# radoslawkrolikowski/financial-market-data-analysis

Measured on AMD Instinct MI355X. Metric: train seq/sec + 3-class acc, biGRU on synthetic order-book, higher is better.
Workload: dtype bf16; 1 GPU; model=biGRU L2 H128 bidirectional, global_batch=8192, seq_len=120, n_features=96, parallelism=dp1, bench_config=repo

## Files before the change

fmda_amd/metrics.py:

```python
from typing import Tuple

import torch


def subset_accuracy(target: torch.Tensor, pred: torch.Tensor) -> torch.Tensor:
    t = target.to(torch.bool)
    p = pred.to(torch.bool)
    return (t == p).all(dim=1).float().mean()


def hamming(target: torch.Tensor, pred: torch.Tensor) -> torch.Tensor:
    t = target.to(torch.bool)
    p = pred.to(torch.bool)
    return (t != p).float().mean()


def fbeta_per_class(target: torch.Tensor, pred: torch.Tensor,
                    beta: float = 0.5) -> torch.Tensor:
    t = target.to(torch.float32)
    p = pred.to(torch.float32)
    tp = (t * p).sum(dim=0)
    fp = ((1 - t) * p).sum(dim=0)
    fn = (t * (1 - p)).sum(dim=0)
    b2 = beta * beta
    denom = (1 + b2) * tp + b2 * fn + fp
    fbeta = torch.where(denom > 0, (1 + b2) * tp / torch.clamp(denom, min=1e-38),
                        torch.zeros_like(denom))
    return fbeta
# ... 32 lines not shown
```

fmda_amd/ops/blas.py:

```python
import os


import torch

_TUNABLE_READY = False


def enable_tunableop() -> bool:
    global _TUNABLE_READY
    if _TUNABLE_READY or not torch.cuda.is_available():
        return _TUNABLE_READY
    try:
        tun = torch.cuda.tunable
        csv = os.path.join(os.path.dirname(__file__), "tunableop_gfx950.csv")
        tune = os.environ.get("FMDA_TUNE", "0") == "1"
        tun.set_filename(csv, insert_device_ordinal=False)
        tun.enable(True)
        tun.tuning_enable(tune)
        _TUNABLE_READY = True
    except Exception:
        _TUNABLE_READY = False
    return _TUNABLE_READY


def chunked_colsum(dg: torch.Tensor, chunks: int = 48) -> torch.Tensor:
    M, N = dg.shape
    c = chunks
    while c > 1 and M % c != 0:
        c //= 2
    if c <= 1:
        return dg.sum(dim=0, dtype=torch.float32)
    return dg.view(c, M // c, N).sum(dim=1, dtype=torch.float32).sum(dim=0)


def chunked_outer(dg: torch.Tensor, x: torch.Tensor,
                  chunks: int = 64, out_fp32: bool = False) -> torch.Tensor:
    parts = chunked_outer_parts(dg, x, chunks)
    if parts.shape[0] == 1:
        return parts[0].float() if out_fp32 else parts[0]
    s = parts.float().sum(dim=0)
    return s if out_fp32 else s.to(dg.dtype)


def chunked_outer_parts(dg: torch.Tensor, x: torch.Tensor,
                        chunks: int = 64) -> torch.Tensor:
    M, N = dg.shape
    K = x.shape[1]
    c = chunks
    while c > 1 and M % c != 0:
        c //= 2
    if c <= 1:
        return torch.matmul(dg.t(), x).unsqueeze(0)
    return torch.bmm(dg.view(c, M // c, N).transpose(1, 2),
                     x.view(c, M // c, K))
```

fmda_amd/ops/csrc/bindings.cpp:

```cpp
#include <torch/extension.h>
#include <ATen/hip/HIPContext.h>

#include <climits>
#include <cstdint>
#include <vector>

extern "C" int fmda_gru_fwd_launch(int is_bf16, int Hp, const void* gi,
                                   const void* w, const float* bhh, void* out,
                                   float* hlast, int B, int Tseq, int n_dir,
                                   const float* h0, void* out_drop,
                                   unsigned int drop_thr, float drop_scale,
                                   unsigned long long drop_seed,
                                   long gi_pitch, hipStream_t stream);
extern "C" int fmda_gru_fwd_cs_launch(const void* gi, const void* w,
                                      const float* bhh, void* out,
                                      float* hlast, void* hpub,
                                      unsigned int* cnt, int B, int Tseq,
                                      int n_dir, void* out_drop,
                                      unsigned int drop_thr,
                                      float drop_scale,
                                      unsigned long long drop_seed,
                                      long gi_pitch, hipStream_t stream);
extern "C" int fmda_gru_bwd_cs_launch(const void* gi, const void* w,
                                      const void* wt, const float* bhh,
// ... 63 lines not shown
                                    float* logits, float* sig,
                                    float* loss_sum, int B, int K, int C,
                                    hipStream_t stream);
extern "C" int fmda_head_bwd_launch(int is_bf16, const float* sig,
                                    const float* y, const float* wgt,
                                    const float* pw, const float* gscale,
                                    const void* W, float* dlogits, void* dx,
                                    int B, int K, int C, hipStream_t stream);
extern "C" int fmda_gru_bwd_db_rows(int is_bf16, int Hp, int B,
                                    int column_split);
extern "C" int fmda_gru_db_reduce_launch(const float* part, int rows,
                                         int n_dir, int Hp, float* dbhh,
                                         float* dbih, hipStream_t stream);
extern "C" int fmda_opt_norm2_launch(const void* chunks, int n_chunks,
                                     float* out, hipStream_t stream);
extern "C" int fmda_pack_gru_layer_launch(
        int is_bf16, const float* const* masters, void* w_ih_cat,
        void* b_ih_cat, void* w_hh_cat, float* b_hh_cat, void* wt, int D,
        int H, int Hp, int F, hipStream_t stream);
extern "C" int fmda_finalize_gru_wgrads_launch(
        int part_bf16, const void* part_ih, int c_ih, const void* part_hh,
        int c_hh, float* const* grads, int D, int H, int Hp, int F,
        hipStream_t stream);
extern "C" int fmda_head_fwd_master_launch(
        int is_bf16, const void* x, const float* W, const float* bias,
        const float* y, const float* wgt, const float* pw, float* logits,
        float* sig, float* loss_sum, int B, int K, int C,
        hipStream_t stream);
extern "C" int fmda_head_bwd_master_launch(
        int is_bf16, const float* sig, const float* y, const float* wgt,
        const float* pw, const float* gscale, const float* W,
        float* dlogits, void* dx, int B, int K, int C, hipStream_t stream);
extern "C" int fmda_normalize_table_launch(
        int out_bf16, const float* x, const float* xmin, const float* xmax,
        void* y, long N, int F, hipStream_t stream);
extern "C" int fmda_window_batch_launch(
        int is_bf16, const void* table, const long* starts, void* out,
        long B, long Tlen, long F, int mode, unsigned int thr, float scale,
        unsigned long long seed, hipStream_t stream);
extern "C" int fmda_head_wgrads_slabs(int B);
extern "C" int fmda_head_wgrads_launch(
        int is_bf16, const float* dlogits, const void* x, float* dw_part,
        float* db_part, float* dW, float* db, int B, int K, int C,
        hipStream_t stream);
namespace fmda_ckpt {
void save_state_dict(const std::string& path,
                     const std::vector<std::string>& keys,
                     const std::vector<torch::Tensor>& tensors);
std::vector<std::pair<std::string, torch::Tensor>> load_state_dict(
        const std::string& path);
}

extern "C" int fmda_opt_adam_launch(const void* chunks, int n_chunks,
                                    const float* norm2, float clip, float lr,
                                    float beta1, float beta2, float eps,
// ... 617 lines not shown
                        torch::IntArrayRef({3 * H, H}) &&
                    masters[4 * d + 2].sizes() == torch::IntArrayRef({3 * H}) &&
                    masters[4 * d + 3].sizes() == torch::IntArrayRef({3 * H}),
                    "pack_gru_layer: master shapes disagree");
        for (int k = 0; k < 4; ++k)
            ptrs[4 * d + k] = masters[4 * d + k].data_ptr<float>();
    }
    const bool bf16 = compute_dtype_is_bf16(dtype);
    auto opt = masters[0].options().dtype(dtype);
    auto w_ih_cat = torch::empty({D * 3 * Hp, F}, opt);
    auto b_ih_cat = torch::empty({D * 3 * Hp}, opt);
    auto w_hh_cat = torch::empty({D, 3 * Hp, Hp}, opt);
    auto b_hh_cat = torch::empty({D, 3 * Hp}, masters[0].options());
    auto wt = torch::empty({D, Hp, 3 * Hp}, opt);
    auto stream = at::hip::getCurrentHIPStream();
    int rc = fmda_pack_gru_layer_launch(
        bf16 ? 1 : 0, ptrs, w_ih_cat.data_ptr(), b_ih_cat.data_ptr(),
        w_hh_cat.data_ptr(), b_hh_cat.data_ptr<float>(), wt.data_ptr(),
        (int)D, (int)H, (int)Hp, (int)F, stream.stream());
    TORCH_CHECK(rc == 0, "pack_gru_layer launch failed");
    return {w_ih_cat, b_ih_cat, w_hh_cat, b_hh_cat, wt};
}

std::vector<torch::Tensor> finalize_gru_wgrads(torch::Tensor part_ih,
                                               torch::Tensor part_hh,
                                               int64_t D, int64_t H,
                                               int64_t Hp) {
    TORCH_CHECK(part_ih.is_cuda() && part_hh.is_cuda() &&
                part_ih.is_contiguous() && part_hh.is_contiguous() &&
                part_ih.dim() == 3 && part_hh.dim() == 3,
                "finalize_gru_wgrads: partials must be contiguous (c, N, K) "
                "GPU tensors");
    TORCH_CHECK(part_ih.scalar_type() == part_hh.scalar_type(),
                "finalize_gru_wgrads: partial dtypes disagree");
    const bool bf16 = compute_dtype_is_bf16(part_ih.scalar_type());
    TORCH_CHECK((D == 1 || D == 2) && H >= 1 && H <= Hp,
                "finalize_gru_wgrads: bad D / H / Hp");
    const int64_t F = part_ih.size(2);
    TORCH_CHECK(part_ih.size(1) == D * 3 * Hp &&
                part_hh.size(1) == D * 3 * Hp && part_hh.size(2) == D * Hp,
                "finalize_gru_wgrads: partial shapes disagree with D / Hp");
    auto f32 = part_ih.options().dtype(torch::kFloat32);
    std::vector<torch::Tensor> grads;
    float* ptrs[4] = {};
    for (int64_t d = 0; d < D; ++d) {
        grads.push_back(torch::empty({3 * H, F}, f32));
        grads.push_back(torch::empty({3 * H, H}, f32));
        ptrs[2 * d] = grads[2 * d].data_ptr<float>();
        ptrs[2 * d + 1] = grads[2 * d + 1].data_ptr<float>();
    }
    auto stream = at::hip::getCurrentHIPStream();
    int rc = fmda_finalize_gru_wgrads_launch(
        bf16 ? 1 : 0, part_ih.data_ptr(), (int)part_ih.size(0),
        part_hh.data_ptr(), (int)part_hh.size(0), ptrs, (int)D, (int)H,
        (int)Hp, (int)F, stream.stream());
    TORCH_CHECK(rc == 0, "finalize_gru_wgrads launch failed");
    return grads;
}

std::vector<torch::Tensor> head_loss_fwd_master(
        torch::Tensor x, torch::Tensor W, torch::Tensor b, torch::Tensor y,
        torch::Tensor wgt, torch::Tensor pw) {
    TORCH_CHECK(x.is_cuda() && x.is_contiguous() && x.dim() == 2);
    const bool bf16 = compute_dtype_is_bf16(x.scalar_type());
    check_f32_cuda(W, "head W"); check_f32_cuda(b, "head b");
    check_f32_cuda(y, "head y"); check_f32_cuda(wgt, "head weight");
    check_f32_cuda(pw, "head pos_weight");
    const int B = x.size(0), K = x.size(1), C = W.size(0);
    TORCH_CHECK(W.size(1) == K && b.numel() == C && y.numel() == (int64_t)B * C
                && wgt.numel() == C && pw.numel() == C,
                "head_loss_fwd_master: shape mismatch");
    auto f32 = x.options().dtype(torch::kFloat32);
    auto logits = torch::empty({B, C}, f32);
    auto sig = torch::empty({B, C}, f32);
    auto part = torch::empty({((int64_t)B * C + 255) / 256}, f32);
    auto stream = at::hip::getCurrentHIPStream();
    int rc = fmda_head_fwd_master_launch(
        bf16 ? 1 : 0, x.data_ptr(), W.data_ptr<float>(), b.data_ptr<float>(),
        y.data_ptr<float>(), wgt.data_ptr<float>(), pw.data_ptr<float>(),
        logits.data_ptr<float>(), sig.data_ptr<float>(),
        part.data_ptr<float>(), B, K, C, stream.stream());
    TORCH_CHECK(rc == 0, "head fwd (master) launch failed");
    return {logits, sig, part.sum().reshape({1})};
}

std::vector<torch::Tensor> head_loss_bwd_master(
        torch::Tensor sig, torch::Tensor y, torch::Tensor wgt,
        torch::Tensor pw, torch::Tensor gscale, torch::Tensor W,
        torch::ScalarType xdtype) {
    check_f32_cuda(sig, "head sig"); check_f32_cuda(y, "head y");
    check_f32_cuda(wgt, "head weight"); check_f32_cuda(pw, "head pos_weight");
    check_f32_cuda(gscale, "head gscale"); check_f32_cuda(W, "head W");
    const int B = sig.size(0), C = sig.size(1), K = W.size(1);
    TORCH_CHECK(W.size(0) == C && y.numel() == sig.numel() &&
                wgt.numel() == C && pw.numel() == C && gscale.numel() == 1,
                "head_loss_bwd_master: shape mismatch");
    const bool bf16 = compute_dtype_is_bf16(xdtype);
    auto dlogits = torch::empty_like(sig);
    auto dx = torch::empty({B, K}, sig.options().dtype(xdtype));
    auto stream = at::hip::getCurrentHIPStream();
    int rc = fmda_head_bwd_master_launch(
        bf16 ? 1 : 0, sig.data_ptr<float>(), y.data_ptr<float>(),
        wgt.data_ptr<float>(), pw.data_ptr<float>(),
        gscale.data_ptr<float>(), W.data_ptr<float>(),
        dlogits.data_ptr<float>(), dx.data_ptr(), B, K, C, stream.stream());
    TORCH_CHECK(rc == 0, "head bwd (master) launch failed");
    return {dlogits, dx};
}

std::vector<torch::Tensor> head_wgrads(torch::Tensor dlogits,
                                       torch::Tensor x) {
    check_f32_cuda(dlogits, "head dlogits");
    TORCH_CHECK(x.is_cuda() && x.is_contiguous() && x.dim() == 2 &&
                dlogits.dim() == 2 && dlogits.size(0) == x.size(0),
                "head_wgrads: shape mismatch");
    const bool bf16 = compute_dtype_is_bf16(x.scalar_type());
    const int B = x.size(0), K = x.size(1), C = dlogits.size(1);
    const int64_t n_slabs = fmda_head_wgrads_slabs(B);
    auto f32 = dlogits.options();
    auto dw_part = torch::empty({n_slabs, C, K}, f32);
    auto db_part = torch::empty({n_slabs, C}, f32);
    auto dW = torch::empty({C, K}, f32);
    auto db = torch::empty({C}, f32);
    auto stream = at::hip::getCurrentHIPStream();
    int rc = fmda_head_wgrads_launch(
        bf16 ? 1 : 0, dlogits.data_ptr<float>(), x.data_ptr(),
        dw_part.data_ptr<float>(), db_part.data_ptr<float>(),
        dW.data_ptr<float>(), db.data_ptr<float>(), B, K, C,
        stream.stream());
    TORCH_CHECK(rc == 0, "head_wgrads launch failed");
// ... 29 lines not shown
    m.def("spatial_dropout_fused", &spatial_dropout_fused,
          "channel (Dropout2d) dropout over (B, T, F) without permutes");
    m.def("ingest_row", &ingest_row,
          "streaming ingest: shift GPU window ring + normalize new row");
    m.def("pool_concat_infer", &pool_concat_infer,
          "fused [dirsum(h_last) | max | avg] concat for inference");
    m.def("head_sigmoid", &head_sigmoid,
          "linear head + sigmoid emitting probabilities");
    m.def("pool_fwd", &pool_fwd, "fused dirsum+max/avg pooling forward",
          py::arg("out"), py::arg("n_dir"), py::arg("act_dtype") = false,
          py::arg("serial") = false);
    m.def("pool_features_fwd", &pool_features_fwd,
          "[dirsum(h_last) | max | avg] features + argmax in one kernel",
          py::arg("out"), py::arg("h_last"));
    m.def("pool_features_bwd", &pool_features_bwd,
          "d_out and d_hlast of pool_features_fwd in one kernel",
          py::arg("dfeat"), py::arg("amax"), py::arg("T"), py::arg("n_dir"));
    m.def("pool_bwd", &pool_bwd, "fused pooling backward (d_out assembly)");
    m.def("head_loss_fwd", &head_loss_fwd, "fused head GEMM + BCE loss");
    m.def("head_loss_bwd", &head_loss_bwd, "fused head/loss backward");
    m.def("pack_gru_layer", &pack_gru_layer,
          "fp32 masters -> padded compute-dtype layer weights (+ W_hh^T)");
    m.def("finalize_gru_wgrads", &finalize_gru_wgrads,
          "split-K partials -> master-shaped fp32 dW_ih / dW_hh");
    m.def("head_loss_fwd_master", &head_loss_fwd_master,
          "fused head GEMM + BCE loss reading the fp32 master W / b");
    m.def("head_loss_bwd_master", &head_loss_bwd_master,
          "fused head/loss backward reading the fp32 master W");
    m.def("head_wgrads", &head_wgrads,
          "head dW / db in fp32, two-stage fixed-order batch reduction");
    m.def("fused_clip_adam", &fused_clip_adam,
          "fused multi-tensor grad-clip + Adam step");
    m.def("save_state_dict_native", &fmda_ckpt::save_state_dict,
          "write a torch.load-compatible zip state_dict (native C++)");
    m.def("load_state_dict_native", &fmda_ckpt::load_state_dict,
          "read a torch.save zip state_dict (native C++)");
}
```

fmda_amd/ops/csrc/glue_kernels.hip:

```cpp
#include <hip/hip_runtime.h>
#include <hip/hip_bf16.h>

#include <cstdint>

#include "dropout_common.h"

#define FMDA_DEV __device__ __forceinline__

namespace fmda {
namespace {

#define FMDA_LOG2E 1.4426950408889634f

FMDA_DEV float fast_exp2(float x) { return __builtin_amdgcn_exp2f(x); }
FMDA_DEV float fast_rcp(float x) { return __builtin_amdgcn_rcpf(x); }
FMDA_DEV float sigmoidf(float x) {
    return fast_rcp(1.0f + fast_exp2(-x * FMDA_LOG2E));
}

template <typename T> FMDA_DEV float to_f32(T v);
template <> FMDA_DEV float to_f32<float>(float v) { return v; }
template <> FMDA_DEV float to_f32<__hip_bfloat16>(__hip_bfloat16 v) {
    return __bfloat162float(v);
}
template <typename T> FMDA_DEV T from_f32(float v);
template <> FMDA_DEV float from_f32<float>(float v) { return v; }
template <> FMDA_DEV __hip_bfloat16 from_f32<__hip_bfloat16>(float v) {
    return __float2bfloat16(v);
}
template <typename T> FMDA_DEV float round_to(float v) {
    return to_f32<T>(from_f32<T>(v));
}

struct GruMasters {
    const float* w_ih[2];
    const float* w_hh[2];
    const float* b_ih[2];
    const float* b_hh[2];
};

template <typename T>
__global__ void pack_gru_layer_kernel(GruMasters m, T* __restrict__ w_ih_cat,
                                      T* __restrict__ b_ih_cat,
                                      T* __restrict__ w_hh_cat,
                                      float* __restrict__ b_hh_cat,
                                      T* __restrict__ wt, int D, int H,
                                      int Hp, int F) {
    const long G3 = 3L * Hp;
    const long n_ih = (long)D * G3 * F;
    const long n_hh = (long)D * G3 * Hp;
    const long n_b = (long)D * G3;
    const long total = n_ih + 2 * n_hh + 2 * n_b;
    const long stride = (long)gridDim.x * blockDim.x;
    for (long i = (long)blockIdx.x * blockDim.x + threadIdx.x; i < total;
         i += stride) {
// ... 58 lines not shown
    const long r = idx % per_dir;
    float acc = 0.0f;
    if (r < n_ih) {
        const int row = (int)(r / F), col = (int)(r % F);
        const long prow = (long)d * 3 * Hp + (long)(row / H) * Hp + row % H;
        const PT* p = part_ih + prow * F + col;
        const long cs = (long)D * 3 * Hp * F;
#pragma unroll 8
        for (int k = 0; k < c_ih; ++k) acc += to_f32<PT>(p[k * cs]);
        o.dw_ih[d][r] = acc;
    } else {
        const long q = r - n_ih;
        const int row = (int)(q / H), col = (int)(q % H);
        const long prow = (long)d * 3 * Hp + (long)(row / H) * Hp + row % H;
        const long pitch = (long)D * Hp;
        const PT* p = part_hh + prow * pitch + (long)d * Hp + col;
        const long cs = (long)D * 3 * Hp * pitch;
#pragma unroll 8
        for (int k = 0; k < c_hh; ++k) acc += to_f32<PT>(p[k * cs]);
        o.dw_hh[d][q] = acc;
    }
}

template <typename T>
__global__ void head_fwd_master_kernel(const T* __restrict__ x,
                                       const float* __restrict__ W,
                                       const float* __restrict__ bias,
                                       const float* __restrict__ y,
                                       const float* __restrict__ wgt,
                                       const float* __restrict__ pw,
                                       float* __restrict__ logits,
                                       float* __restrict__ sig,
                                       float* __restrict__ loss_sum, int B,
                                       int K, int C) {
    const int idx = blockIdx.x * blockDim.x + threadIdx.x;
    float l = 0.0f;
    if (idx < B * C) {
        const int r = idx / C, c = idx % C;
        const T* xr = x + (long)r * K;
        const float* wr = W + (long)c * K;
        float acc = round_to<T>(bias[c]);
        for (int k = 0; k < K; ++k)
            acc += to_f32<T>(xr[k]) * round_to<T>(wr[k]);
        logits[idx] = acc;
        const float s = sigmoidf(acc);
        sig[idx] = s;
        const float yy = y[idx];
        const float m = acc > 0.0f ? acc : 0.0f;
        const float lse = m + __builtin_logf(fast_exp2(-m * FMDA_LOG2E) +
                                             fast_exp2((acc - m) * FMDA_LOG2E));
        const float log_s = acc - lse;
        const float log_1ms = -lse;
        l = -wgt[c] * (pw[c] * yy * log_s + (1.0f - yy) * log_1ms);
    }
    __shared__ float red[4];
    float v = l;
    v += __shfl_xor(v, 1); v += __shfl_xor(v, 2); v += __shfl_xor(v, 4);
    v += __shfl_xor(v, 8); v += __shfl_xor(v, 16); v += __shfl_xor(v, 32);
    if ((threadIdx.x & 63) == 0) red[threadIdx.x >> 6] = v;
    __syncthreads();
    if (threadIdx.x == 0) {
        float t = 0.0f;
        for (int w = 0; w < (int)(blockDim.x >> 6); ++w) t += red[w];
        loss_sum[blockIdx.x] = t;
    }
}

template <typename T>
__global__ void head_bwd_master_kernel(const float* __restrict__ sig,
                                       const float* __restrict__ y,
                                       const float* __restrict__ wgt,
                                       const float* __restrict__ pw,
                                       const float* __restrict__ gscale,
                                       const float* __restrict__ W,
                                       float* __restrict__ dlogits,
                                       T* __restrict__ dx, int B, int K,
                                       int C) {
    const int idx = blockIdx.x * blockDim.x + threadIdx.x;
    if (idx >= B * K) return;
    const int r = idx / K, k = idx % K;
    const float g = *gscale / (float)(B * C);
    float acc = 0.0f;
    for (int c = 0; c < C; ++c) {
        const float s = sig[r * C + c];
        const float yy = y[r * C + c];
        const float dl = g * wgt[c] * (s * (1.0f - yy + pw[c] * yy) -
                                       pw[c] * yy);
        if (k == 0) dlogits[r * C + c] = dl;
        acc += dl * round_to<T>(W[(long)c * K + k]);
    }
    dx[idx] = from_f32<T>(acc);
}

constexpr int HEAD_SLAB = 64;

struct CompSum {
    float s = 0.0f, c = 0.0f;
    FMDA_DEV void add(float v) {
#pragma clang fp contract(off)
        const float t = s + v;
        c += fabsf(s) >= fabsf(v) ? (s - t) + v : (v - t) + s;
        s = t;
    }
    FMDA_DEV float value() const { return s + c; }
};

template <typename T>
__global__ void head_wgrads_stage1_kernel(const float* __restrict__ dlogits,
                                          const T* __restrict__ x,
                                          float* __restrict__ dw_part,
                                          float* __restrict__ db_part, int B,
// ... 19 lines not shown
    if (k == 0) db_part[slab * C + c] = db.value();
}

__global__ void head_wgrads_stage2_kernel(const float* __restrict__ dw_part,
                                          const float* __restrict__ db_part,
                                          float* __restrict__ dW,
                                          float* __restrict__ db, int n_slabs,
                                          int K, int C) {
    const int idx = blockIdx.x * blockDim.x + threadIdx.x;
    const int n_w = C * K;
    if (idx >= n_w + C) return;
    CompSum a;
    if (idx < n_w) {
#pragma unroll 8
        for (int s = 0; s < n_slabs; ++s) a.add(dw_part[(long)s * n_w + idx]);
        dW[idx] = a.value();
    } else {
        const int c = idx - n_w;
        for (int s = 0; s < n_slabs; ++s) a.add(db_part[s * C + c]);
        db[c] = a.value();
    }
}

template <typename T>
__global__ void normalize_table_kernel(const float* __restrict__ x,
                                       const float* __restrict__ xmin,
                                       const float* __restrict__ xmax,
                                       T* __restrict__ y, long total, int F) {
    const long stride = (long)gridDim.x * blockDim.x;
    for (long i = (long)blockIdx.x * blockDim.x + threadIdx.x; i < total;
         i += stride) {
        const int f = (int)(i % F);
        float v = x[i];
        if (v != v) v = 0.0f;
        else if (v == __builtin_inff()) v = 3.402823466e+38f;
        else if (v == -__builtin_inff()) v = -3.402823466e+38f;
        const float mn = xmin[f];
        y[i] = from_f32<T>(__fdiv_rn(__fsub_rn(v, mn), __fsub_rn(xmax[f], mn)));
    }
}

struct alignas(16) chunk16 { unsigned int u[4]; };

template <int LB>
FMDA_DEV void load16(void* dst, const void* src) {
    if constexpr (LB == 16) {
        *(chunk16*)dst = *(const chunk16*)src;
    } else if constexpr (LB == 8) {
        ((uint2*)dst)[0] = ((const uint2*)src)[0];
        ((uint2*)dst)[1] = ((const uint2*)src)[1];
    } else {
        static_assert(LB == 4, "load16: LB is 16, 8 or 4");
#pragma unroll
        for (int k = 0; k < 4; ++k)
            ((unsigned int*)dst)[k] = ((const unsigned int*)src)[k];
    }
}

template <typename T, int LB, int MODE>
__global__ void window_batch_kernel(const T* __restrict__ table,
                                    const long* __restrict__ starts,
                                    T* __restrict__ out, long n, long TF,
                                    int F, unsigned int thr, float scale,
                                    unsigned long long seed) {
    constexpr int V = 16 / (int)sizeof(T);
// ... 116 lines not shown

extern "C" int fmda_finalize_gru_wgrads_launch(
        int part_bf16, const void* part_ih, int c_ih, const void* part_hh,
        int c_hh, float* const* grads, int D, int H, int Hp, int F,
        hipStream_t stream) {
    GruWgrads o = {};
    for (int d = 0; d < D; ++d) {
        o.dw_ih[d] = grads[2 * d + 0];
        o.dw_hh[d] = grads[2 * d + 1];
    }
    const long total = (long)D * 3 * H * ((long)F + H);
    const dim3 grid((unsigned)((total + 255) / 256));
    if (part_bf16)
        finalize_gru_wgrads_kernel<__hip_bfloat16><<<grid, 256, 0, stream>>>(
            (const __hip_bfloat16*)part_ih, c_ih,
            (const __hip_bfloat16*)part_hh, c_hh, o, D, H, Hp, F);
    else
        finalize_gru_wgrads_kernel<float><<<grid, 256, 0, stream>>>(
            (const float*)part_ih, c_ih, (const float*)part_hh, c_hh, o, D,
            H, Hp, F);
    return launch_ok();
}

extern "C" int fmda_head_fwd_master_launch(
        int is_bf16, const void* x, const float* W, const float* bias,
        const float* y, const float* wgt, const float* pw, float* logits,
        float* sig, float* loss_sum, int B, int K, int C,
        hipStream_t stream) {
    const dim3 grid((B * C + 255) / 256);
    if (is_bf16)
        head_fwd_master_kernel<__hip_bfloat16><<<grid, 256, 0, stream>>>(
            (const __hip_bfloat16*)x, W, bias, y, wgt, pw, logits, sig,
            loss_sum, B, K, C);
    else
        head_fwd_master_kernel<float><<<grid, 256, 0, stream>>>(
            (const float*)x, W, bias, y, wgt, pw, logits, sig, loss_sum, B,
            K, C);
    return launch_ok();
}

extern "C" int fmda_head_bwd_master_launch(
        int is_bf16, const float* sig, const float* y, const float* wgt,
        const float* pw, const float* gscale, const float* W,
        float* dlogits, void* dx, int B, int K, int C, hipStream_t stream) {
    const dim3 grid((B * K + 255) / 256);
    if (is_bf16)
        head_bwd_master_kernel<__hip_bfloat16><<<grid, 256, 0, stream>>>(
            sig, y, wgt, pw, gscale, W, dlogits, (__hip_bfloat16*)dx, B, K,
            C);
    else
        head_bwd_master_kernel<float><<<grid, 256, 0, stream>>>(
            sig, y, wgt, pw, gscale, W, dlogits, (float*)dx, B, K, C);
    return launch_ok();
}

extern "C" int fmda_normalize_table_launch(
        int out_bf16, const float* x, const float* xmin, const float* xmax,
        void* y, long N, int F, hipStream_t stream) {
    const long total = N * (long)F;
    if (total == 0) return 0;
    const long blocks = (total + 255) / 256;
    const dim3 grid((unsigned)(blocks < 4096 ? blocks : 4096));
    if (out_bf16)
        normalize_table_kernel<__hip_bfloat16><<<grid, 256, 0, stream>>>(
            x, xmin, xmax, (__hip_bfloat16*)y, total, F);
    else
        normalize_table_kernel<float><<<grid, 256, 0, stream>>>(
            x, xmin, xmax, (float*)y, total, F);
    return launch_ok();
}

extern "C" int fmda_window_batch_load_bytes(const void* table, long TF,
                                            long F, int es) {
    if (TF % (16 / es) != 0) return 0;
    const uintptr_t addr = (uintptr_t)table;
// ... 59 lines not shown
```

fmda_amd/ops/interface.py:

```python
import os
from typing import List, Optional, Tuple

import torch

from . import load_extension
from .blas import (chunked_colsum, chunked_outer, chunked_outer_parts,
                   enable_tunableop)

_ALLOWED_HP = [32, 64, 128, 256, 512]


def _pad_h(H: int) -> int:
    for hp in _ALLOWED_HP:
        if H <= hp:
            return hp
    raise ValueError(f"hidden size {H} > {_ALLOWED_HP[-1]} not supported")


def _glue_mode() -> int:
    return {"0": 0, "2": 2}.get(os.environ.get("FMDA_NATIVE_GLUE", "1"), 1)


def _native_glue() -> bool:
    return _glue_mode() >= 1


def _native_reductions() -> bool:
    return _glue_mode() == 2


def _fp32_cuda(*tensors) -> bool:
    return all(t.is_cuda and t.dtype == torch.float32 for t in tensors)


def _pad_gate_rows(w: torch.Tensor, H: int, Hp: int) -> torch.Tensor:
    if H == Hp:
        return w
    shape = list(w.shape)
    shape[0] = 3 * Hp
    out = w.new_zeros(shape)
    for g in range(3):
        out[g * Hp:g * Hp + H] = w[g * H:(g + 1) * H]
    return out


def _pad_cols(w: torch.Tensor, H: int, Hp: int) -> torch.Tensor:
    if H == Hp:
        return w
    shape = list(w.shape)
    shape[-1] = Hp
    out = w.new_zeros(shape)
# ... 262 lines not shown

    @staticmethod
    def backward(ctx, dloss, _dlogits):
        ext = load_extension()
        x2d, W, y, wgt, pw, sig = ctx.saved_tensors
        dlogits, dx = ext.head_loss_bwd(sig, y, wgt, pw,
                                        dloss.reshape(1).float().contiguous(),
                                        W, x2d.dtype)
        dl = dlogits.to(x2d.dtype)
        dW = chunked_outer(dl, x2d)
        db = dlogits.sum(dim=0).to(W.dtype)
        return dx, dW, db, None, None, None


class _HeadLossMaster(torch.autograd.Function):

    @staticmethod
    def forward(ctx, x2d, W, b, y, wgt, pw):
        ext = load_extension()
        ctx.native_reductions = _native_reductions()
        x2d = x2d.contiguous()
        W = W.contiguous()
        y, wgt, pw = y.contiguous(), wgt.contiguous(), pw.contiguous()
        logits, sig, loss_sum = ext.head_loss_fwd_master(
            x2d, W, b.contiguous(), y, wgt, pw)
        B, C = logits.shape
        loss = (loss_sum / float(B * C)).reshape(())
        ctx.save_for_backward(x2d, W, y, wgt, pw, sig)
        ctx.mark_non_differentiable(logits)
        return loss, logits

    @staticmethod
    def backward(ctx, dloss, _dlogits):
        ext = load_extension()
        x2d, W, y, wgt, pw, sig = ctx.saved_tensors
        dlogits, dx = ext.head_loss_bwd_master(
            sig, y, wgt, pw, dloss.reshape(1).float().contiguous(), W,
            x2d.dtype)
        if ctx.native_reductions:
            dW, db = ext.head_wgrads(dlogits, x2d)
        else:
            dW = chunked_outer(dlogits.to(x2d.dtype), x2d).to(W.dtype)
            db = dlogits.sum(dim=0).to(x2d.dtype).to(W.dtype)
        return dx, dW, db, None, None, None


def fused_head_loss(x2d, weight, bias, y, wgt, pw):
    if (_native_glue() and x2d.is_cuda and _fp32_cuda(weight, bias)
            and x2d.dtype in (torch.bfloat16, torch.float32)):
        return _HeadLossMaster.apply(x2d, weight, bias, y.float(),
                                     wgt.float(), pw.float())
    Wc = weight.to(x2d.dtype)
    bc = bias.to(x2d.dtype)
    return _HeadLoss.apply(x2d, Wc, bc, y.float(), wgt.float(), pw.float())


def _unpad_gate_rows(w, H, Hp):
    if H == Hp:
        return w
    return torch.cat([w[g * Hp:g * Hp + H] for g in range(3)], dim=0)


class _BiGRULayer(torch.autograd.Function):

# ... 2 lines not shown
                w_ih1, w_hh1, b_ih1, b_hh1, out_drop_p=0.0,
                out_drop_seed=0, h0=None):
        ext = load_extension()
        D = 2 if w_ih1 is not None else 1
        H = w_hh0.shape[1]
        dtype = x.dtype
        B, T, F = x.shape
        params = [(w_ih0, w_hh0, b_ih0, b_hh0)]
        if D == 2:
            params.append((w_ih1, w_hh1, b_ih1, b_hh1))
        with torch.no_grad():
            w_ih_cat, b_ih_cat, w_hh_cat, b_hh_cat, wt = _pack_layer(
                params, H, Hp, dtype)
        x2d = x.reshape(B * T, F)
        gi = torch.addmm(b_ih_cat, x2d, w_ih_cat.t()).view(B, T, -1)
        h0c = h0.detach().contiguous() if h0 is not None else None
        res = ext.gru_fwd(gi, w_hh_cat, b_hh_cat, h0c, out_drop_p,
                          out_drop_seed)
        out, h_last = res[0], res[1]
        ctx.save_for_backward(x2d, w_ih_cat, w_hh_cat, b_hh_cat, gi, out, wt)
        ctx.h0 = h0c
        ctx.meta = (D, H, Hp, out_drop_p, out_drop_seed)
        ctx.native_reductions = _native_reductions()
        ctx.set_materialize_grads(False)
        if len(res) > 2:
            return out, h_last, res[2]
        return out, h_last

    @staticmethod
    def backward(ctx, d_out, d_hlast, d_outdrop=None):
        ext = load_extension()
        x2d, w_ih_cat, w_hh_cat, b_hh_cat, gi, out, wt = ctx.saved_tensors
        D, H, Hp, drop_p, drop_seed = ctx.meta
        need_dx = ctx.needs_input_grad[0]
        if drop_p > 0:
            assert d_out is None, "unexpected grad on raw out with fused dropout"
            d_out = d_outdrop
        if d_out is None:
            d_out = torch.zeros_like(out)
        if d_hlast is None:
            d_hlast = out.new_zeros(
                (w_hh_cat.shape[0], out.shape[0], Hp), dtype=torch.float32)
        d_out = d_out.contiguous().to(gi.dtype)
        d_hlast = d_hlast.contiguous().float()
        h0c = ctx.h0
        res = ext.gru_bwd(gi, w_hh_cat, b_hh_cat, out, d_out, d_hlast,
                          drop_p, drop_seed, h0c, wt)
        dgi, dgh, dh0_out, dbhh, dbih = res[:5]
        dgh0 = res[5] if len(res) > 5 else None
        M = dgi.shape[0] * dgi.shape[1]
        dx = None
        if need_dx:
            dx = torch.matmul(dgi.reshape(M, -1), w_ih_cat)
            dx = dx.view(dgi.shape[0], dgi.shape[1], -1)
        dh0_grad = dh0_out if h0c is not None else None

        if wt is not None and ctx.native_reductions and dgh0 is None:
            wg = ext.finalize_gru_wgrads(
                chunked_outer_parts(dgi.reshape(M, -1), x2d),
                chunked_outer_parts(dgh.reshape(M, -1), out.reshape(M, -1)),
                D, H, Hp)
            wgrads = [(wg[2 * d], wg[2 * d + 1]) for d in range(D)]
        else:
            cross = chunked_outer(dgh.reshape(M, -1), out.reshape(M, -1),
                                  out_fp32=True)
            if dgh0 is not None:
                for d in range(D):
                    cross[d * 3 * Hp:(d + 1) * 3 * Hp,
                          d * Hp:(d + 1) * Hp] += dgh0[d].float().t() @ h0c[d]
            dwih_cat = chunked_outer(dgi.reshape(M, -1), x2d, out_fp32=True)
            wgrads = []
            for d in range(D):
                dwih = dwih_cat[d * 3 * Hp:(d + 1) * 3 * Hp]
                dwhh = cross[d * 3 * Hp:(d + 1) * 3 * Hp,
                             d * Hp:(d + 1) * Hp].contiguous()
                wgrads.append((_unpad_gate_rows(dwih, H, Hp),
                               _unpad_gate_rows(dwhh, H, Hp)[:, :H]))

        grads = [wgrads[d] + (_unpad_gate_rows(dbih[d], H, Hp),
                              _unpad_gate_rows(dbhh[d], H, Hp))
                 for d in range(D)]
        if D == 1:
            grads.append((None, None, None, None))
        (a0, b0, c0, e0), (a1, b1, c1, e1) = grads
# ... 166 lines not shown
```

Baseline: 1.064 million seq/s.

## Add fused eager-order wgrad reductions, staged head forward, and native subset accuracy

Adds custom kernels that reduce the 64 split-K GEMM partials into master-shaped fp32 GRU and head weight gradients in one pass. The summation order mirrors the eager chunked sum so results stay bit-identical, and it replaces the chain of float cast, sum, slice and unpad ops. The head forward gains an LDS-staged variant that tiles x and W into shared memory, and the head backward can emit a bf16 copy of dlogits directly. Subset accuracy becomes a single-block kernel. These trim launch count and memory traffic in the glue path, at the cost of several shape-specific code paths.

```diff
diff --git a/fmda_amd/metrics.py b/fmda_amd/metrics.py
--- a/fmda_amd/metrics.py
+++ b/fmda_amd/metrics.py
@@ -4,6 +4,17 @@
 
 
 def subset_accuracy(target: torch.Tensor, pred: torch.Tensor) -> torch.Tensor:
+    if (target.is_cuda and pred.is_cuda and pred.dtype == torch.bool
+            and target.dtype in (torch.float32, torch.bool)
+            and target.dim() == 2 and target.shape == pred.shape
+            and target.device == pred.device
+            and 1 <= target.shape[0] <= 65536
+            and 1 <= target.shape[1] <= 65536
+            and target.is_contiguous() and pred.is_contiguous()):
+        from .ops import load_extension
+        from .ops.interface import _native_glue
+        if _native_glue():
+            return load_extension().subset_accuracy(target, pred)
     t = target.to(torch.bool)
     p = pred.to(torch.bool)
     return (t == p).all(dim=1).float().mean()
diff --git a/fmda_amd/ops/blas.py b/fmda_amd/ops/blas.py
--- a/fmda_amd/ops/blas.py
+++ b/fmda_amd/ops/blas.py
@@ -42,13 +42,18 @@
     return s if out_fp32 else s.to(dg.dtype)
 
 
+def split_chunks(M: int, chunks: int = 64) -> int:
+    c = chunks
+    while c > 1 and M % c != 0:
+        c //= 2
+    return max(c, 1)
+
+
 def chunked_outer_parts(dg: torch.Tensor, x: torch.Tensor,
                         chunks: int = 64) -> torch.Tensor:
     M, N = dg.shape
     K = x.shape[1]
-    c = chunks
-    while c > 1 and M % c != 0:
-        c //= 2
+    c = split_chunks(M, chunks)
     if c <= 1:
         return torch.matmul(dg.t(), x).unsqueeze(0)
     return torch.bmm(dg.view(c, M // c, N).transpose(1, 2),
diff --git a/fmda_amd/ops/csrc/bindings.cpp b/fmda_amd/ops/csrc/bindings.cpp
--- a/fmda_amd/ops/csrc/bindings.cpp
+++ b/fmda_amd/ops/csrc/bindings.cpp
@@ -109,15 +109,27 @@
         int part_bf16, const void* part_ih, int c_ih, const void* part_hh,
         int c_hh, float* const* grads, int D, int H, int Hp, int F,
         hipStream_t stream);
+extern "C" int fmda_finalize_gru_wgrads_eager_launch(
+        int part_bf16, const void* part_ih, const void* part_hh,
+        float* const* grads, int D, int H, int Hp, int F,
+        hipStream_t stream);
+extern "C" int fmda_eager_sum_chunks();
+extern "C" int fmda_head_wgrads_eager_launch(
+        int is_bf16, const void* parts, const float* db_sum, float* dW,
+        float* db, int K, int C, hipStream_t stream);
+extern "C" int fmda_subset_accuracy_launch(
+        int target_is_float, const void* target, const void* pred,
+        float* out, int B, int C, hipStream_t stream);
 extern "C" int fmda_head_fwd_master_launch(
         int is_bf16, const void* x, const float* W, const float* bias,
         const float* y, const float* wgt, const float* pw, float* logits,
-        float* sig, float* loss_sum, int B, int K, int C,
+        float* sig, float* loss_sum, int B, int K, int C, int staged,
         hipStream_t stream);
 extern "C" int fmda_head_bwd_master_launch(
         int is_bf16, const float* sig, const float* y, const float* wgt,
         const float* pw, const float* gscale, const float* W,
-        float* dlogits, void* dx, int B, int K, int C, hipStream_t stream);
+        float* dlogits, void* dlogits_t, void* dx, int B, int K, int C,
+        hipStream_t stream);
 extern "C" int fmda_normalize_table_launch(
         int out_bf16, const float* x, const float* xmin, const float* xmax,
         void* y, long N, int F, hipStream_t stream);
@@ -781,10 +793,19 @@
     return {w_ih_cat, b_ih_cat, w_hh_cat, b_hh_cat, wt};
 }
 
+bool eager_sum_applies(torch::Tensor parts) {
+    if (parts.dim() != 3 || parts.size(0) != fmda_eager_sum_chunks())
+        return false;
+    const int64_t outputs = parts.size(1) * parts.size(2);
+    return outputs >= 512 && outputs % 4 == 0;
+}
+
+
 std::vector<torch::Tensor> finalize_gru_wgrads(torch::Tensor part_ih,
                                                torch::Tensor part_hh,
                                                int64_t D, int64_t H,
-                                               int64_t Hp) {
+                                               int64_t Hp,
+                                               bool eager_order) {
     TORCH_CHECK(part_ih.is_cuda() && part_hh.is_cuda() &&
                 part_ih.is_contiguous() && part_hh.is_contiguous() &&
                 part_ih.dim() == 3 && part_hh.dim() == 3,
@@ -809,17 +830,27 @@
         ptrs[2 * d + 1] = grads[2 * d + 1].data_ptr<float>();
     }
     auto stream = at::hip::getCurrentHIPStream();
-    int rc = fmda_finalize_gru_wgrads_launch(
-        bf16 ? 1 : 0, part_ih.data_ptr(), (int)part_ih.size(0),
-        part_hh.data_ptr(), (int)part_hh.size(0), ptrs, (int)D, (int)H,
-        (int)Hp, (int)F, stream.stream());
+    int rc;
+    if (eager_order) {
+        TORCH_CHECK(eager_sum_applies(part_ih) && eager_sum_applies(part_hh),
+                    "finalize_gru_wgrads: the eager sum order is known only "
+                    "for 64 chunks of >= 512 outputs, a multiple of 4");
+        rc = fmda_finalize_gru_wgrads_eager_launch(
+            bf16 ? 1 : 0, part_ih.data_ptr(), part_hh.data_ptr(), ptrs,
+            (int)D, (int)H, (int)Hp, (int)F, stream.stream());
+    } else {
+        rc = fmda_finalize_gru_wgrads_launch(
+            bf16 ? 1 : 0, part_ih.data_ptr(), (int)part_ih.size(0),
+            part_hh.data_ptr(), (int)part_hh.size(0), ptrs, (int)D, (int)H,
+            (int)Hp, (int)F, stream.stream());
+    }
     TORCH_CHECK(rc == 0, "finalize_gru_wgrads launch failed");
     return grads;
 }
 
 std::vector<torch::Tensor> head_loss_fwd_master(
         torch::Tensor x, torch::Tensor W, torch::Tensor b, torch::Tensor y,
-        torch::Tensor wgt, torch::Tensor pw) {
+        torch::Tensor wgt, torch::Tensor pw, bool staged) {
     TORCH_CHECK(x.is_cuda() && x.is_contiguous() && x.dim() == 2);
     const bool bf16 = compute_dtype_is_bf16(x.scalar_type());
     check_f32_cuda(W, "head W"); check_f32_cuda(b, "head b");
@@ -838,15 +869,15 @@
         bf16 ? 1 : 0, x.data_ptr(), W.data_ptr<float>(), b.data_ptr<float>(),
         y.data_ptr<float>(), wgt.data_ptr<float>(), pw.data_ptr<float>(),
         logits.data_ptr<float>(), sig.data_ptr<float>(),
-        part.data_ptr<float>(), B, K, C, stream.stream());
+        part.data_ptr<float>(), B, K, C, staged ? 1 : 0, stream.stream());
     TORCH_CHECK(rc == 0, "head fwd (master) launch failed");
-    return {logits, sig, part.sum().reshape({1})};
+    return {logits, sig, part.sum().reshape({1}), part};
 }
 
 std::vector<torch::Tensor> head_loss_bwd_master(
         torch::Tensor sig, torch::Tensor y, torch::Tensor wgt,
         torch::Tensor pw, torch::Tensor gscale, torch::Tensor W,
-        torch::ScalarType xdtype) {
+        torch::ScalarType xdtype, bool emit_cast) {
     check_f32_cuda(sig, "head sig"); check_f32_cuda(y, "head y");
     check_f32_cuda(wgt, "head weight"); check_f32_cuda(pw, "head pos_weight");
     check_f32_cuda(gscale, "head gscale"); check_f32_cuda(W, "head W");
@@ -857,14 +888,63 @@
     const bool bf16 = compute_dtype_is_bf16(xdtype);
     auto dlogits = torch::empty_like(sig);
     auto dx = torch::empty({B, K}, sig.options().dtype(xdtype));
+    torch::Tensor dl_t;
+    if (emit_cast && bf16)
+        dl_t = torch::empty({B, C}, sig.options().dtype(xdtype));
     auto stream = at::hip::getCurrentHIPStream();
     int rc = fmda_head_bwd_master_launch(
         bf16 ? 1 : 0, sig.data_ptr<float>(), y.data_ptr<float>(),
         wgt.data_ptr<float>(), pw.data_ptr<float>(),
         gscale.data_ptr<float>(), W.data_ptr<float>(),
-        dlogits.data_ptr<float>(), dx.data_ptr(), B, K, C, stream.stream());
+        dlogits.data_ptr<float>(), dl_t.defined() ? dl_t.data_ptr() : nullptr,
+        dx.data_ptr(), B, K, C, stream.stream());
     TORCH_CHECK(rc == 0, "head bwd (master) launch failed");
-    return {dlogits, dx};
+    if (!emit_cast) return {dlogits, dx};
+    return {dlogits, dx, bf16 ? dl_t : dlogits};
+}
+
+std::vector<torch::Tensor> head_wgrads_eager(torch::Tensor parts,
+                                             torch::Tensor db_sum) {
+    TORCH_CHECK(parts.is_cuda() && parts.is_contiguous() &&
+                eager_sum_applies(parts),
+                "head_wgrads_eager: parts must be contiguous (64, C, K) GPU "
+                "partials with C*K >= 512, a multiple of 4");
+    check_f32_cuda(db_sum, "head db_sum");
+    const bool bf16 = compute_dtype_is_bf16(parts.scalar_type());
+    const int C = parts.size(1), K = parts.size(2);
+    TORCH_CHECK(db_sum.numel() == C && db_sum.is_contiguous(),
+                "head_wgrads_eager: shape mismatch");
+    auto f32 = db_sum.options();
+    auto dW = torch::empty({C, K}, f32);
+    auto db = torch::empty({C}, f32);
+    auto stream = at::hip::getCurrentHIPStream();
+    int rc = fmda_head_wgrads_eager_launch(
+        bf16 ? 1 : 0, parts.data_ptr(), db_sum.data_ptr<float>(),
+        dW.data_ptr<float>(), db.data_ptr<float>(), K, C, stream.stream());
+    TORCH_CHECK(rc == 0, "head_wgrads_eager launch failed");
+    return {dW, db};
+}
+
+torch::Tensor subset_accuracy(torch::Tensor target, torch::Tensor pred) {
+    TORCH_CHECK(target.is_cuda() && pred.is_cuda() && target.dim() == 2 &&
+                target.sizes() == pred.sizes() && target.is_contiguous() &&
+                pred.is_contiguous() && pred.scalar_type() == torch::kBool &&
+                target.device() == pred.device(),
+                "subset_accuracy: need contiguous (B, C) GPU tensors, pred "
+                "bool");
+    const bool tf = target.scalar_type() == torch::kFloat32;
+    TORCH_CHECK(tf || target.scalar_type() == torch::kBool,
+                "subset_accuracy: target must be fp32 or bool");
+    const int64_t B = target.size(0), C = target.size(1);
+    TORCH_CHECK(B >= 1 && B <= (1 << 16) && C >= 1 && C <= (1 << 16),
+                "subset_accuracy: 1 <= B, C <= 65536");
+    auto out = torch::empty({}, target.options().dtype(torch::kFloat32));
+    auto stream = at::hip::getCurrentHIPStream();
+    int rc = fmda_subset_accuracy_launch(
+        tf ? 1 : 0, target.data_ptr(), pred.data_ptr(),
+        out.data_ptr<float>(), (int)B, (int)C, stream.stream());
+    TORCH_CHECK(rc == 0, "subset_accuracy launch failed");
+    return out;
 }
 
 std::vector<torch::Tensor> head_wgrads(torch::Tensor dlogits,
@@ -940,11 +1020,25 @@
     m.def("pack_gru_layer", &pack_gru_layer,
           "fp32 masters -> padded compute-dtype layer weights (+ W_hh^T)");
     m.def("finalize_gru_wgrads", &finalize_gru_wgrads,
-          "split-K partials -> master-shaped fp32 dW_ih / dW_hh");
+          "split-K partials -> master-shaped fp32 dW_ih / dW_hh",
+          py::arg("part_ih"), py::arg("part_hh"), py::arg("D"), py::arg("H"),
+          py::arg("Hp"), py::arg("eager_order") = false);
+    m.def("eager_sum_applies", &eager_sum_applies,
+          "whether the eager chunk-sum order is known for these partials");
     m.def("head_loss_fwd_master", &head_loss_fwd_master,
-          "fused head GEMM + BCE loss reading the fp32 master W / b");
+          "fused head GEMM + BCE loss reading the fp32 master W / b; "
+          "returns (logits, sig, loss_sum, block partials)",
+          py::arg("x"), py::arg("W"), py::arg("b"), py::arg("y"),
+          py::arg("wgt"), py::arg("pw"), py::arg("staged") = true);
     m.def("head_loss_bwd_master", &head_loss_bwd_master,
-          "fused head/loss backward reading the fp32 master W");
+          "fused head/loss backward reading the fp32 master W",
+          py::arg("sig"), py::arg("y"), py::arg("wgt"), py::arg("pw"),
+          py::arg("gscale"), py::arg("W"), py::arg("xdtype"),
+          py::arg("emit_cast") = false);
+    m.def("head_wgrads_eager", &head_wgrads_eager,
+          "head dW / db from the split-K partials, the eager chain's bits");
+    m.def("subset_accuracy", &subset_accuracy,
+          "exact-match ratio of a (B, C) multilabel batch in one kernel");
     m.def("head_wgrads", &head_wgrads,
           "head dW / db in fp32, two-stage fixed-order batch reduction");
     m.def("fused_clip_adam", &fused_clip_adam,
diff --git a/fmda_amd/ops/csrc/glue_kernels.hip b/fmda_amd/ops/csrc/glue_kernels.hip
--- a/fmda_amd/ops/csrc/glue_kernels.hip
+++ b/fmda_amd/ops/csrc/glue_kernels.hip
@@ -31,6 +31,7 @@
 template <typename T> FMDA_DEV float round_to(float v) {
     return to_f32<T>(from_f32<T>(v));
 }
+struct alignas(16) chunk16 { unsigned int u[4]; };
 
 struct GruMasters {
     const float* w_ih[2];
@@ -135,6 +136,92 @@
     }
 }
 
+constexpr int EAGER_SUM_CHUNKS = 64;
+
+template <int BYTES> struct raw_vec;
+template <> struct raw_vec<2> { using type = unsigned short; };
+template <> struct raw_vec<4> { using type = unsigned int; };
+template <> struct raw_vec<8> { using type = uint2; };
+template <> struct raw_vec<16> { using type = uint4; };
+
+template <typename PT, int V>
+FMDA_DEV void eager_order_sum64(const PT* __restrict__ p, long cs,
+                                float (&out)[V]) {
+    using raw_t = typename raw_vec<V * (int)sizeof(PT)>::type;
+    float row[2][V];
+#pragma unroll
+    for (int y = 0; y < 2; ++y) {
+        float a[4][V];
+#pragma unroll
+        for (int i = 0; i < 4; ++i)
+#pragma unroll
+            for (int j = 0; j < V; ++j) a[i][j] = 0.0f;
+#pragma unroll
+        for (int n = 0; n < EAGER_SUM_CHUNKS / 8; ++n) {
+#pragma unroll
+            for (int i = 0; i < 4; ++i) {
+                alignas(V * sizeof(PT)) PT v[V];
+                *(raw_t*)v = *(const raw_t*)(p + (y + 2 * (4 * n + i)) * cs);
+#pragma unroll
+                for (int j = 0; j < V; ++j) a[i][j] += to_f32<PT>(v[j]);
+            }
+        }
+#pragma unroll
+        for (int j = 0; j < V; ++j)
+            row[y][j] = ((a[0][j] + a[1][j]) + a[2][j]) + a[3][j];
+    }
+#pragma unroll
+    for (int j = 0; j < V; ++j) out[j] = row[0][j] + row[1][j];
+}
+
+template <typename PT, int V>
+__global__ void __launch_bounds__(256) finalize_gru_wgrads_eager_kernel(
+        const PT* __restrict__ part_ih, const PT* __restrict__ part_hh,
+        GruWgrads o, int D, int H, int Hp, int F) {
+    const long n_ih = 3L * H * F;
+    const long n_hh = 3L * H * H;
+    const long per_dir = n_ih + n_hh;
+    const long idx = ((long)blockIdx.x * blockDim.x + threadIdx.x) * V;
+    if (idx >= (long)D * per_dir) return;
+    const int d = (int)(idx / per_dir);
+    const long r = idx % per_dir;
+    float acc[V];
+    float* dst;
+    if (r < n_ih) {
+        const int row = (int)(r / F), col = (int)(r % F);
+        const long prow = (long)d * 3 * Hp + (long)(row / H) * Hp + row % H;
+        eager_order_sum64<PT, V>(part_ih + prow * F + col,
+                                 (long)D * 3 * Hp * F, acc);
+        dst = o.dw_ih[d] + r;
+    } else {
+        const long q = r - n_ih;
+        const int row = (int)(q / H), col = (int)(q % H);
+        const long prow = (long)d * 3 * Hp + (long)(row / H) * Hp + row % H;
+        const long pitch = (long)D * Hp;
+        eager_order_sum64<PT, V>(part_hh + prow * pitch + (long)d * Hp + col,
+                                 (long)D * 3 * Hp * pitch, acc);
+        dst = o.dw_hh[d] + q;
+    }
+#pragma unroll
+    for (int j = 0; j < V; ++j) dst[j] = acc[j];
+}
+
+template <typename T>
+__global__ void head_wgrads_eager_kernel(const T* __restrict__ parts,
+                                         const float* __restrict__ db_sum,
+                                         float* __restrict__ dW,
+                                         float* __restrict__ db, int n_w,
+                                         int C) {
+    const int idx = blockIdx.x * blockDim.x + threadIdx.x;
+    if (idx < n_w) {
+        float s[1];
+        eager_order_sum64<T, 1>(parts + idx, (long)n_w, s);
+        dW[idx] = round_to<T>(s[0]);
+    } else if (idx < n_w + C) {
+        db[idx - n_w] = round_to<T>(db_sum[idx - n_w]);
+    }
+}
+
 template <typename T>
 __global__ void head_fwd_master_kernel(const T* __restrict__ x,
                                        const float* __restrict__ W,
@@ -180,6 +267,86 @@
 }
 
 template <typename T>
+__global__ void head_fwd_master_staged_kernel(
+        const T* __restrict__ x, const float* __restrict__ W,
+        const float* __restrict__ bias, const float* __restrict__ y,
+        const float* __restrict__ wgt, const float* __restrict__ pw,
+        float* __restrict__ logits, float* __restrict__ sig,
+        float* __restrict__ loss_sum, int B, int K, int C, int KT,
+        int rows_cap) {
+    constexpr int V = 16 / (int)sizeof(T);
+    extern __shared__ __align__(16) unsigned char head_smem[];
+    const int xpitch = KT * (int)sizeof(T) + 16;
+    const int wpitch = KT + 4;
+    unsigned char* xs = head_smem;
+    float* ws = (float*)(head_smem + (size_t)rows_cap * xpitch);
+
+    const int first = blockIdx.x * blockDim.x;
+    const int idx = first + threadIdx.x;
+    const int last = min(first + (int)blockDim.x, B * C) - 1;
+    const int r0 = first / C;
+    const int nrows = last / C - r0 + 1;
+    const bool valid = idx < B * C;
+    const int r = valid ? idx / C : r0, c = valid ? idx % C : 0;
+    float acc = round_to<T>(bias[c]);
+    for (int k0 = 0; k0 < K; k0 += KT) {
+        const int kt = min(KT, K - k0);
+        const int cpr = kt / V;
+        if (k0 > 0) __syncthreads();
+        for (int j = threadIdx.x; j < nrows * cpr; j += blockDim.x) {
+            const int row = j / cpr, cc = j % cpr;
+            *(chunk16*)(xs + row * xpitch + cc * 16) =
+                *(const chunk16*)(x + (long)(r0 + row) * K + k0 + cc * V);
+        }
+        for (int j = threadIdx.x; j < C * kt; j += blockDim.x) {
+            const int cw = j / kt, kk = j % kt;
+            ws[cw * wpitch + kk] = round_to<T>(W[(long)cw * K + k0 + kk]);
+        }
+        __syncthreads();
+        if (valid) {
+            const unsigned char* xr = xs + (r - r0) * xpitch;
+            const float* wr = ws + c * wpitch;
+            for (int kk = 0; kk < kt; kk += V) {
+                alignas(16) T xv[V];
+                alignas(16) float wv[V];
+                *(chunk16*)xv = *(const chunk16*)(xr + kk * (int)sizeof(T));
+#pragma unroll
+                for (int q = 0; q < V / 4; ++q)
+                    *(chunk16*)(wv + 4 * q) =
+                        *(const chunk16*)(wr + kk + 4 * q);
+#pragma unroll
+                for (int j = 0; j < V; ++j)
+                    acc = __builtin_fmaf(to_f32<T>(xv[j]), wv[j], acc);
+            }
+        }
+    }
+    float l = 0.0f;
+    if (valid) {
+        logits[idx] = acc;
+        const float s = sigmoidf(acc);
+        sig[idx] = s;
+        const float yy = y[idx];
+        const float m = acc > 0.0f ? acc : 0.0f;
+        const float lse = m + __builtin_logf(fast_exp2(-m * FMDA_LOG2E) +
+                                             fast_exp2((acc - m) * FMDA_LOG2E));
+        const float log_s = acc - lse;
+        const float log_1ms = -lse;
+        l = -wgt[c] * (pw[c] * yy * log_s + (1.0f - yy) * log_1ms);
+    }
+    __shared__ float red[4];
+    float v = l;
+    v += __shfl_xor(v, 1); v += __shfl_xor(v, 2); v += __shfl_xor(v, 4);
+    v += __shfl_xor(v, 8); v += __shfl_xor(v, 16); v += __shfl_xor(v, 32);
+    if ((threadIdx.x & 63) == 0) red[threadIdx.x >> 6] = v;
+    __syncthreads();
+    if (threadIdx.x == 0) {
+        float t = 0.0f;
+        for (int w = 0; w < (int)(blockDim.x >> 6); ++w) t += red[w];
+        loss_sum[blockIdx.x] = t;
+    }
+}
+
+template <typename T>
 __global__ void head_bwd_master_kernel(const float* __restrict__ sig,
                                        const float* __restrict__ y,
                                        const float* __restrict__ wgt,
@@ -187,6 +354,7 @@
                                        const float* __restrict__ gscale,
                                        const float* __restrict__ W,
                                        float* __restrict__ dlogits,
+                                       T* __restrict__ dlogits_t,
                                        T* __restrict__ dx, int B, int K,
                                        int C) {
     const int idx = blockIdx.x * blockDim.x + threadIdx.x;
@@ -199,7 +367,10 @@
         const float yy = y[r * C + c];
         const float dl = g * wgt[c] * (s * (1.0f - yy + pw[c] * yy) -
                                        pw[c] * yy);
-        if (k == 0) dlogits[r * C + c] = dl;
+        if (k == 0) {
+            dlogits[r * C + c] = dl;
+            if (dlogits_t != nullptr) dlogits_t[r * C + c] = from_f32<T>(dl);
+        }
         acc += dl * round_to<T>(W[(long)c * K + k]);
     }
     dx[idx] = from_f32<T>(acc);
@@ -265,6 +436,35 @@
     }
 }
 
+constexpr int SUBSET_ACC_THREADS = 1024;
+
+template <typename TT>
+__global__ void subset_accuracy_kernel(const TT* __restrict__ target,
+                                       const unsigned char* __restrict__ pred,
+                                       float* __restrict__ out, int B, int C,
+                                       float inv_b) {
+    int cnt = 0;
+    for (int r = threadIdx.x; r < B; r += blockDim.x) {
+        const TT* t = target + (long)r * C;
+        const unsigned char* p = pred + (long)r * C;
+        bool all = true;
+        for (int c = 0; c < C; ++c)
+            all = all && ((t[c] != (TT)0) == (p[c] != 0));
+        cnt += all ? 1 : 0;
+    }
+    cnt += __shfl_xor(cnt, 1); cnt += __shfl_xor(cnt, 2);
+    cnt += __shfl_xor(cnt, 4); cnt += __shfl_xor(cnt, 8);
+    cnt += __shfl_xor(cnt, 16); cnt += __shfl_xor(cnt, 32);
+    __shared__ int red[SUBSET_ACC_THREADS / 64];
+    if ((threadIdx.x & 63) == 0) red[threadIdx.x >> 6] = cnt;
+    __syncthreads();
+    if (threadIdx.x == 0) {
+        int total = 0;
+        for (int w = 0; w < (int)(blockDim.x >> 6); ++w) total += red[w];
+        out[0] = (float)total * inv_b;
+    }
+}
+
 template <typename T>
 __global__ void normalize_table_kernel(const float* __restrict__ x,
                                        const float* __restrict__ xmin,
@@ -283,7 +483,6 @@
     }
 }
 
-struct alignas(16) chunk16 { unsigned int u[4]; };
 
 template <int LB>
 FMDA_DEV void load16(void* dst, const void* src) {
@@ -446,12 +645,101 @@
     return launch_ok();
 }
 
+extern "C" int fmda_finalize_gru_wgrads_eager_launch(
+        int part_bf16, const void* part_ih, const void* part_hh,
+        float* const* grads, int D, int H, int Hp, int F,
+        hipStream_t stream) {
+    GruWgrads o = {};
+    for (int d = 0; d < D; ++d) {
+        o.dw_ih[d] = grads[2 * d + 0];
+        o.dw_hh[d] = grads[2 * d + 1];
+    }
+    const long total = (long)D * 3 * H * ((long)F + H);
+    const bool vec = H % 4 == 0 && F % 4 == 0;
+    const long threads = vec ? total / 4 : total;
+    const dim3 grid((unsigned)((threads + 255) / 256));
+#define FMDA_FIN(PT, V)                                                    \
+    finalize_gru_wgrads_eager_kernel<PT, V><<<grid, 256, 0, stream>>>(     \
+        (const PT*)part_ih, (const PT*)part_hh, o, D, H, Hp, F)
+    if (part_bf16) {
+        if (vec) FMDA_FIN(__hip_bfloat16, 4);
+        else FMDA_FIN(__hip_bfloat16, 1);
+    } else {
+        if (vec) FMDA_FIN(float, 4);
+        else FMDA_FIN(float, 1);
+    }
+#undef FMDA_FIN
+    return launch_ok();
+}
+
+extern "C" int fmda_eager_sum_chunks() { return EAGER_SUM_CHUNKS; }
+
+extern "C" int fmda_head_wgrads_eager_launch(
+        int is_bf16, const void* parts, const float* db_sum, float* dW,
+        float* db, int K, int C, hipStream_t stream) {
+    const int n_w = C * K;
+    const dim3 grid((n_w + C + 255) / 256);
+    if (is_bf16)
+        head_wgrads_eager_kernel<__hip_bfloat16><<<grid, 256, 0, stream>>>(
+            (const __hip_bfloat16*)parts, db_sum, dW, db, n_w, C);
+    else
+        head_wgrads_eager_kernel<float><<<grid, 256, 0, stream>>>(
+            (const float*)parts, db_sum, dW, db, n_w, C);
+    return launch_ok();
+}
+
+extern "C" int fmda_subset_accuracy_launch(
+        int target_is_float, const void* target, const void* pred,
+        float* out, int B, int C, hipStream_t stream) {
+    const float inv_b = 1.0f / (float)B;
+    if (target_is_float)
+        subset_accuracy_kernel<float><<<1, SUBSET_ACC_THREADS, 0, stream>>>(
+            (const float*)target, (const unsigned char*)pred, out, B, C,
+            inv_b);
+    else
+        subset_accuracy_kernel<unsigned char>
+            <<<1, SUBSET_ACC_THREADS, 0, stream>>>(
+                (const unsigned char*)target, (const unsigned char*)pred,
+                out, B, C, inv_b);
+    return launch_ok();
+}
+
+static int head_fwd_stage_tile(const void* x, int es, int B, int K, int C,
+                               int* rows_cap) {
+    const int V = 16 / es;
+    if (B < 1 || C < 1 || K % V != 0 || (uintptr_t)x % 16 != 0) return 0;
+    const int rc = 255 / C + 2 < B ? 255 / C + 2 : B;
+    const long budget = 64512 - 16L * rc - 16L * C;
+    long kt = budget / ((long)rc * es + 4L * C);
+    if (kt > K) kt = K;
+    if (kt < K) kt -= kt % 8;
+    *rows_cap = rc;
+    return kt >= 8 || kt == K ? (int)kt : 0;
+}
+
 extern "C" int fmda_head_fwd_master_launch(
         int is_bf16, const void* x, const float* W, const float* bias,
         const float* y, const float* wgt, const float* pw, float* logits,
-        float* sig, float* loss_sum, int B, int K, int C,
+        float* sig, float* loss_sum, int B, int K, int C, int staged,
         hipStream_t stream) {
     const dim3 grid((B * C + 255) / 256);
+    int rows_cap = 0;
+    const int es = is_bf16 ? 2 : 4;
+    const int kt = staged ? head_fwd_stage_tile(x, es, B, K, C, &rows_cap) : 0;
+    if (kt > 0) {
+        const size_t lds = (size_t)rows_cap * (kt * es + 16) +
+                           (size_t)C * (kt + 4) * 4;
+        if (is_bf16)
+            head_fwd_master_staged_kernel<__hip_bfloat16>
+                <<<grid, 256, lds, stream>>>(
+                    (const __hip_bfloat16*)x, W, bias, y, wgt, pw, logits,
+                    sig, loss_sum, B, K, C, kt, rows_cap);
+        else
+            head_fwd_master_staged_kernel<float><<<grid, 256, lds, stream>>>(
+                (const float*)x, W, bias, y, wgt, pw, logits, sig, loss_sum,
+                B, K, C, kt, rows_cap);
+        return launch_ok();
+    }
     if (is_bf16)
         head_fwd_master_kernel<__hip_bfloat16><<<grid, 256, 0, stream>>>(
             (const __hip_bfloat16*)x, W, bias, y, wgt, pw, logits, sig,
@@ -466,15 +754,17 @@
 extern "C" int fmda_head_bwd_master_launch(
         int is_bf16, const float* sig, const float* y, const float* wgt,
         const float* pw, const float* gscale, const float* W,
-        float* dlogits, void* dx, int B, int K, int C, hipStream_t stream) {
+        float* dlogits, void* dlogits_t, void* dx, int B, int K, int C,
+        hipStream_t stream) {
     const dim3 grid((B * K + 255) / 256);
     if (is_bf16)
         head_bwd_master_kernel<__hip_bfloat16><<<grid, 256, 0, stream>>>(
-            sig, y, wgt, pw, gscale, W, dlogits, (__hip_bfloat16*)dx, B, K,
-            C);
+            sig, y, wgt, pw, gscale, W, dlogits, (__hip_bfloat16*)dlogits_t,
+            (__hip_bfloat16*)dx, B, K, C);
     else
         head_bwd_master_kernel<float><<<grid, 256, 0, stream>>>(
-            sig, y, wgt, pw, gscale, W, dlogits, (float*)dx, B, K, C);
+            sig, y, wgt, pw, gscale, W, dlogits, (float*)dlogits_t,
+            (float*)dx, B, K, C);
     return launch_ok();
 }
 
diff --git a/fmda_amd/ops/interface.py b/fmda_amd/ops/interface.py
--- a/fmda_amd/ops/interface.py
+++ b/fmda_amd/ops/interface.py
@@ -5,7 +5,7 @@
 
 from . import load_extension
 from .blas import (chunked_colsum, chunked_outer, chunked_outer_parts,
-                   enable_tunableop)
+                   enable_tunableop, split_chunks)
 
 _ALLOWED_HP = [32, 64, 128, 256, 512]
 
@@ -27,6 +27,10 @@
 
 def _native_reductions() -> bool:
     return _glue_mode() == 2
+
+
+def _eager_sum_known(M: int, outputs: int) -> bool:
+    return split_chunks(M) == 64 and outputs >= 512 and outputs % 4 == 0
 
 
 def _fp32_cuda(*tensors) -> bool:
@@ -335,7 +339,7 @@
         x2d = x2d.contiguous()
         W = W.contiguous()
         y, wgt, pw = y.contiguous(), wgt.contiguous(), pw.contiguous()
-        logits, sig, loss_sum = ext.head_loss_fwd_master(
+        logits, sig, loss_sum, _ = ext.head_loss_fwd_master(
             x2d, W, b.contiguous(), y, wgt, pw)
         B, C = logits.shape
         loss = (loss_sum / float(B * C)).reshape(())
@@ -347,12 +351,19 @@
     def backward(ctx, dloss, _dlogits):
         ext = load_extension()
         x2d, W, y, wgt, pw, sig = ctx.saved_tensors
-        dlogits, dx = ext.head_loss_bwd_master(
-            sig, y, wgt, pw, dloss.reshape(1).float().contiguous(), W,
-            x2d.dtype)
+        gscale = dloss.reshape(1).float().contiguous()
         if ctx.native_reductions:
+            dlogits, dx = ext.head_loss_bwd_master(sig, y, wgt, pw, gscale,
+                                                   W, x2d.dtype)
             dW, db = ext.head_wgrads(dlogits, x2d)
+        elif _eager_sum_known(x2d.shape[0], W.numel()):
+            dlogits, dx, dl = ext.head_loss_bwd_master(
+                sig, y, wgt, pw, gscale, W, x2d.dtype, True)
+            dW, db = ext.head_wgrads_eager(chunked_outer_parts(dl, x2d),
+                                           dlogits.sum(dim=0))
         else:
+            dlogits, dx = ext.head_loss_bwd_master(sig, y, wgt, pw, gscale,
+                                                   W, x2d.dtype)
             dW = chunked_outer(dlogits.to(x2d.dtype), x2d).to(W.dtype)
             db = dlogits.sum(dim=0).to(x2d.dtype).to(W.dtype)
         return dx, dW, db, None, None, None
@@ -401,6 +412,7 @@
         ctx.h0 = h0c
         ctx.meta = (D, H, Hp, out_drop_p, out_drop_seed)
         ctx.native_reductions = _native_reductions()
+        ctx.native_glue = _native_glue()
         ctx.set_materialize_grads(False)
         if len(res) > 2:
             return out, h_last, res[2]
@@ -439,6 +451,15 @@
                 chunked_outer_parts(dgi.reshape(M, -1), x2d),
                 chunked_outer_parts(dgh.reshape(M, -1), out.reshape(M, -1)),
                 D, H, Hp)
+            wgrads = [(wg[2 * d], wg[2 * d + 1]) for d in range(D)]
+        elif (ctx.native_glue and dgh0 is None
+              and dgi.dtype in (torch.bfloat16, torch.float32)
+              and _eager_sum_known(M, D * 3 * Hp * x2d.shape[1])
+              and _eager_sum_known(M, D * 3 * Hp * D * Hp)):
+            wg = ext.finalize_gru_wgrads(
+                chunked_outer_parts(dgi.reshape(M, -1), x2d),
+                chunked_outer_parts(dgh.reshape(M, -1), out.reshape(M, -1)),
+                D, H, Hp, True)
             wgrads = [(wg[2 * d], wg[2 * d + 1]) for d in range(D)]
         else:
             cross = chunked_outer(dgh.reshape(M, -1), out.reshape(M, -1),
```

Result: faster. 1.089 million seq/s, median of 6 (+2.4%).
